# thygate/stable-diffusion-webui-depthmap-script

Measured on NVIDIA H100. Metric: images/sec, higher is better.
Workload: dtype fp16

## Files before the change

### stable-diffusion-webui-depthmap-script_b200/csrc/gemm_wgmma.cu

```cuda
#include <cuda.h>
#include <cuda_fp16.h>
#include <math.h>
#include <stdlib.h>

#include "common.cuh"
#include "tc_common.cuh"

namespace dm {
using namespace tc;

enum GemmEpi : int {
    EPI_STORE_F16 = 0,
    EPI_RESID_F32 = 1,
    EPI_PIXSHUF = 2,
    EPI_HEAD = 3,
    EPI_STORE_F32 = 4,
};
enum GemmAct : int { ACT_NONE = 0, ACT_GELU = 1, ACT_RELU = 2 };

struct GemmParams {
    int M, N, K;
    int epi, act;
    const float *bias;
    __half *C; int ldc;
    __half *C2;
    const __half *R; int ldr;
    const __half *R2; int ldr2;
    float *X; int ldx;
    const float *gamma;
    float head_b2;
    int ps_s, ps_cout, ps_h, ps_w;
    int cB, cH, cW, cCin, hbox, wbox, tiles_x, tiles_y;
    int m_tiles, n_tiles, group_m;
    int corg;
    const float *wscale;
};

template <int BM, int BN>
struct GemmCfg {
    static constexpr int BK = 64;
    static constexpr int WM = BM / 64;
    static constexpr int A_BYTES = BM * BK * 2, B_BYTES = BN * BK * 2;
    static constexpr int STAGE_BYTES = A_BYTES + B_BYTES;
    static constexpr int STAGES = (220 * 1024) / STAGE_BYTES < 8 ? (220 * 1024) / STAGE_BYTES : 8;
    static constexpr int SMEM_BYTES = STAGES * STAGE_BYTES + 256 ;
};
constexpr int GEMM_THREADS = 384;
constexpr int SPLIT_PROMOTE = 1;

__device__ __forceinline__ float gelu_erf(float x) {
    const float u = fminf(fabsf(x), 5.75f);
    float q = -2.992472582263872e-05f;
    q = fmaf(q, u, 0.0007398786256089807f);
    q = fmaf(q, u, -0.007977476343512535f);
    q = fmaf(q, u, 0.05323820561170578f);
    q = fmaf(q, u, 0.45891568064689636f);
    q = fmaf(q, u, 1.1511471271514893f);
    float e;
    const float t = fmaf(-u, q, -1.f);
    asm("ex2.approx.ftz.f32 %0, %1;" : "=f"(e) : "f"(t));
    return fmaf(-u, e, fmaxf(x, 0.f));
}

__device__ __forceinline__ void split_store2(__half *dst, int lo_off, float v0, float v1) {
    const __half2 hi = __floats2half2_rn(v0, v1);
    const float2 hf = __half22float2(hi);
    const __half2 lo = __floats2half2_rn(v0 - hf.x, v1 - hf.y);
    *reinterpret_cast<__half2 *>(dst) = hi;
    *reinterpret_cast<__half2 *>(dst + lo_off) = lo;
    *reinterpret_cast<__half2 *>(dst + 2 * lo_off) = hi;
}

template <int BN, int EPI, bool SPLIT = false>
__device__ __forceinline__ void epilogue_fragment(const GemmParams &p, const float (&acc)[BN / 2], const long long (&m)[2], const bool (&row_ok)[2],
                                                  int n_base, int lane) {
    constexpr int JC = 2;
    const int t = lane & 3;
    float head_acc[2] = {0.f, 0.f};
#pragma unroll
    for (int j0 = 0; j0 < BN / 8; j0 += JC) {
        float2 b2[JC], g2[JC], x[JC][2], ws[JC];
        __half2 rv[JC][2], rv2[JC][2], rl[JC][2], rl2[JC][2];
#pragma unroll
        for (int jj = 0; jj < JC; ++jj) {
            const int n = n_base + 8 * (j0 + jj) + 2 * t;
            b2[jj] = make_float2(0.f, 0.f);
            g2[jj] = make_float2(0.f, 0.f);
            if (n >= p.N) continue;
            if (p.bias) b2[jj] = __ldg(reinterpret_cast<const float2 *>(p.bias + n));
            if (SPLIT) ws[jj] = __ldg(reinterpret_cast<const float2 *>(p.wscale + n));
            if (EPI == EPI_RESID_F32 || EPI == EPI_HEAD) g2[jj] = __ldg(reinterpret_cast<const float2 *>(p.gamma + n));
#pragma unroll
            for (int r = 0; r < 2; ++r) {
                if (!row_ok[r]) continue;
                if (EPI == EPI_RESID_F32) x[jj][r] = *reinterpret_cast<const float2 *>(p.X + m[r] * p.ldx + n);
                if (EPI == EPI_STORE_F16 || EPI == EPI_PIXSHUF) {
                    if (p.R) rv[jj][r] = __ldg(reinterpret_cast<const __half2 *>(p.R + m[r] * p.ldr + n));
                    if (p.R2) rv2[jj][r] = __ldg(reinterpret_cast<const __half2 *>(p.R2 + m[r] * p.ldr2 + n));
                    if (SPLIT && p.R) rl[jj][r] = __ldg(reinterpret_cast<const __half2 *>(p.R + m[r] * p.ldr + p.N + n));
                    if (SPLIT && p.R2) rl2[jj][r] = __ldg(reinterpret_cast<const __half2 *>(p.R2 + m[r] * p.ldr2 + p.N + n));
                }
            }
        }
#pragma unroll
        for (int jj = 0; jj < JC; ++jj) {
            const int j = j0 + jj;
            const int n = n_base + 8 * j + 2 * t;
            if (n >= p.N) continue;
#pragma unroll
            for (int r = 0; r < 2; ++r) {
                if (!row_ok[r]) continue;
                float v0, v1;
                if (SPLIT) { v0 = fmaf(acc[4 * j + 2 * r], ws[jj].x, b2[jj].x); v1 = fmaf(acc[4 * j + 2 * r + 1], ws[jj].y, b2[jj].y); }
                else { v0 = acc[4 * j + 2 * r] + b2[jj].x; v1 = acc[4 * j + 2 * r + 1] + b2[jj].y; }
                if (EPI == EPI_RESID_F32) {
                    float2 xv = x[jj][r];
                    xv.x = fmaf(g2[jj].x, v0, xv.x); xv.y = fmaf(g2[jj].y, v1, xv.y);
                    *reinterpret_cast<float2 *>(p.X + m[r] * p.ldx + n) = xv;
                    continue;
                }
                if (EPI == EPI_STORE_F32) {
                    *reinterpret_cast<float2 *>(p.X + m[r] * p.ldx + n) = make_float2(v0, v1);
                    continue;
                }
                if (p.act == ACT_GELU) { v0 = gelu_erf(v0); v1 = gelu_erf(v1); }
                else if (p.act == ACT_RELU) { v0 = fmaxf(v0, 0.f); v1 = fmaxf(v1, 0.f); }
                if (EPI == EPI_HEAD) {
                    head_acc[r] = fmaf(v1, g2[jj].y, fmaf(v0, g2[jj].x, head_acc[r]));
                    continue;
                }
                if (SPLIT) {
                    if (p.R) { const float2 f = __half22float2(rv[jj][r]), l = __half22float2(rl[jj][r]); v0 += f.x + l.x; v1 += f.y + l.y; }
                    if (p.R2) { const float2 f = __half22float2(rv2[jj][r]), l = __half22float2(rl2[jj][r]); v0 += f.x + l.x; v1 += f.y + l.y; }
                    __half *dst;
                    int lo_off;
                    if (EPI == EPI_PIXSHUF) {
                        const int s = p.ps_s, ij = n / p.ps_cout, co = n % p.ps_cout;
                        const int i = ij / s, jx = ij % s;
                        const long long bb = m[r] / ((long long)p.ps_h * p.ps_w);
                        const int rem = (int)(m[r] % ((long long)p.ps_h * p.ps_w));
                        const int y = rem / p.ps_w, xx = rem % p.ps_w;
                        dst = p.C + (((bb * (p.ps_h * s) + (y * s + i)) * (long long)(p.ps_w * s)) + (xx * s + jx)) * (3 * p.ps_cout) + co;
                        lo_off = p.ps_cout;
                    } else {
                        dst = p.C + m[r] * p.ldc + n;
                        lo_off = p.N;
                    }
                    split_store2(dst, lo_off, v0, v1);
                    if (EPI != EPI_PIXSHUF && p.C2) split_store2(p.C2 + m[r] * p.ldc + n, lo_off, fmaxf(v0, 0.f), fmaxf(v1, 0.f));
                    continue;
                }
                if (p.R) { const float2 f = __half22float2(rv[jj][r]); v0 += f.x; v1 += f.y; }
                if (p.R2) { const float2 f = __half22float2(rv2[jj][r]); v0 += f.x; v1 += f.y; }
                const __half2 h2 = __floats2half2_rn(v0, v1);
                if (EPI == EPI_PIXSHUF) {
                    const int s = p.ps_s, ij = n / p.ps_cout, co = n % p.ps_cout;
                    const int i = ij / s, jx = ij % s;
                    const long long bb = m[r] / ((long long)p.ps_h * p.ps_w);
                    const int rem = (int)(m[r] % ((long long)p.ps_h * p.ps_w));
                    const int y = rem / p.ps_w, xx = rem % p.ps_w;
                    *reinterpret_cast<__half2 *>(p.C + (((bb * (p.ps_h * s) + (y * s + i)) * (long long)(p.ps_w * s)) + (xx * s + jx)) * p.ps_cout + co) = h2;
                } else {
                    *reinterpret_cast<__half2 *>(p.C + m[r] * p.ldc + n) = h2;
                    if (p.C2) *reinterpret_cast<__half2 *>(p.C2 + m[r] * p.ldc + n) = __hmax2(h2, __float2half2_rn(0.f));
                }
            }
        }
    }
    if (EPI == EPI_HEAD) {
#pragma unroll
        for (int r = 0; r < 2; ++r) {
            float s = head_acc[r];
            s += __shfl_xor_sync(0xffffffffu, s, 1);
            s += __shfl_xor_sync(0xffffffffu, s, 2);
            if (t == 0 && row_ok[r]) p.X[m[r]] = fmaxf(s + p.head_b2, 0.f);
        }
    }
}

__device__ __forceinline__ void tile_coords(const GemmParams &p, int t, int &m_blk, int &n_blk) {
    const int per_group = p.group_m * p.n_tiles;
    const int g = t / per_group, r = t - g * per_group;
    m_blk = g * p.group_m + r / p.n_tiles;
    n_blk = r % p.n_tiles;
}

__device__ __forceinline__ void conv_origin(const GemmParams &p, int m_blk, int &cb, int &cy0, int &cx0) {
    const int tiles_per_img = p.tiles_x * p.tiles_y;
    cb = m_blk / tiles_per_img;
    const int t = m_blk % tiles_per_img;
    cy0 = (t / p.tiles_x) * p.hbox;
    cx0 = (t % p.tiles_x) * p.wbox;
}

template <int BM, int BN, bool CONV, bool SPLIT>
__device__ __forceinline__ void gemm_body(const CUtensorMap &tmA, const CUtensorMap &tmB, const GemmParams &p) {
    using Cfg = GemmCfg<BM, BN>;
    extern __shared__ __align__(1024) uint8_t smem_raw[];
    uint8_t *smem = smem_raw;
    uint64_t *full = reinterpret_cast<uint64_t *>(smem + Cfg::STAGES * Cfg::STAGE_BYTES);
    uint64_t *empty = full + Cfg::STAGES;

    const int warp = threadIdx.x >> 5, lane = threadIdx.x & 31;
    const int num_kb = CONV ? 9 * (p.cCin / Cfg::BK) : p.K / Cfg::BK;
    const int my_tiles = (p.m_tiles * p.n_tiles - (int)blockIdx.x + (int)gridDim.x - 1) / (int)gridDim.x;

    if (threadIdx.x == 0) {
        prefetch_tmap(&tmA);
        prefetch_tmap(&tmB);
        for (int s = 0; s < Cfg::STAGES; ++s) { mbar_init(&full[s], 1); mbar_init(&empty[s], 4); }
        fence_barrier_init();
    }
    __syncthreads();

    if (warp < 4) {
        setmaxnreg_dec<40>();
        if (threadIdx.x == 0) {
            int stage = 0, phase = 0;
            for (int i = 0; i < my_tiles; ++i) {
                int m_blk, n_blk, cb = 0, cy0 = 0, cx0 = 0;
                tile_coords(p, blockIdx.x + i * gridDim.x, m_blk, n_blk);
                if (CONV) conv_origin(p, m_blk, cb, cy0, cx0);
                for (int kb = 0; kb < num_kb; ++kb) {
                    mbar_wait(&empty[stage], phase ^ 1);
                    uint8_t *sa = smem + stage * Cfg::STAGE_BYTES, *sb = sa + Cfg::A_BYTES;
                    mbar_arrive_expect_tx(&full[stage], Cfg::STAGE_BYTES);
                    if (CONV) {
                        const int cblks = p.cCin / Cfg::BK;
                        const int tap = kb / cblks, cblk = kb % cblks;
                        const int dy = tap / 3 - 1, dx = tap % 3 - 1;
                        tma_load_4d(sa, &tmA, &full[stage], cblk * Cfg::BK, cx0 + dx + p.corg, cy0 + dy + p.corg, cb);
                    } else {
                        tma_load_2d(sa, &tmA, &full[stage], kb * Cfg::BK, m_blk * BM);
                    }
                    tma_load_2d(sb, &tmB, &full[stage], kb * Cfg::BK, n_blk * BN);
                    if (++stage == Cfg::STAGES) { stage = 0; phase ^= 1; }
                }
            }
        }
        return;
    }

    setmaxnreg_inc<232>();
    const int wg = (warp >> 2) - 1;
    float acc[Cfg::WM][BN / 2];
    float sum[Cfg::WM][BN / 2];
    for (int i = wg; i < my_tiles; i += 2) {
        int m_blk, n_blk, cb = 0, cy0 = 0, cx0 = 0;
        tile_coords(p, blockIdx.x + i * gridDim.x, m_blk, n_blk);
        if (CONV) conv_origin(p, m_blk, cb, cy0, cx0);
        const long long q0 = (long long)i * num_kb;
        int stage = (int)(q0 % Cfg::STAGES), phase = (int)((q0 / Cfg::STAGES) & 1), prev = 0;
        if (i > 0) named_bar_sync(1 + wg, 256);
        if (SPLIT) {
#pragma unroll
            for (int h = 0; h < Cfg::WM; ++h)
#pragma unroll
                for (int e = 0; e < BN / 2; ++e) sum[h][e] = 0.f;
        }
        for (int kb = 0; kb < num_kb; ++kb) {
            mbar_wait(&full[stage], phase);
            const uint32_t sa = smem_u32(smem + stage * Cfg::STAGE_BYTES), sb = sa + Cfg::A_BYTES;
            const uint64_t bdesc = make_desc_kmajor_sw128(sb);
            wgmma_fence();
#pragma unroll
            for (int k = 0; k < Cfg::BK / 16; ++k) {
#pragma unroll
                for (int h = 0; h < Cfg::WM; ++h)
                    wgmma_ss<BN>(acc[h], make_desc_kmajor_sw128(sa + h * (64 * 128)) + (uint64_t)(2 * k), bdesc + (uint64_t)(2 * k),
                                 SPLIT ? ((kb % SPLIT_PROMOTE) | k) != 0 : (kb | k) != 0);
            }
            wgmma_commit();
            if (kb > 0) {
                wgmma_wait<1>();
                if (lane == 0) mbar_arrive(&empty[prev]);
            }
            if (SPLIT && ((kb + 1) % SPLIT_PROMOTE == 0 || kb + 1 == num_kb)) {
                wgmma_wait<0>();
#pragma unroll
                for (int h = 0; h < Cfg::WM; ++h)
#pragma unroll
                    for (int e = 0; e < BN / 2; ++e) sum[h][e] = __fadd_rn(sum[h][e], acc[h][e]);
            }
            prev = stage;
            if (++stage == Cfg::STAGES) { stage = 0; phase ^= 1; }
        }
        if (i + 1 < my_tiles) named_bar_arrive(2 - wg, 256);
        wgmma_wait<0>();
        if (lane == 0) mbar_arrive(&empty[prev]);

#pragma unroll
        for (int h = 0; h < Cfg::WM; ++h) {
            long long m[2];
            bool row_ok[2];
#pragma unroll
            for (int r = 0; r < 2; ++r) {
                const int row = h * 64 + (warp & 3) * 16 + (lane >> 2) + 8 * r;
                if (CONV) {
                    const int y = cy0 + row / p.wbox, x = cx0 + row % p.wbox;
                    row_ok[r] = (y < p.cH) && (x < p.cW);
                    m[r] = ((long long)cb * p.cH + y) * p.cW + x;
                } else {
                    m[r] = (long long)m_blk * BM + row;
                    row_ok[r] = m[r] < p.M;
                }
            }
            const float (&res)[BN / 2] = SPLIT ? sum[h] : acc[h];
            switch (p.epi) {
                case EPI_STORE_F16: epilogue_fragment<BN, EPI_STORE_F16, SPLIT>(p, res, m, row_ok, n_blk * BN, lane); break;
                case EPI_RESID_F32: epilogue_fragment<BN, EPI_RESID_F32, SPLIT>(p, res, m, row_ok, n_blk * BN, lane); break;
                case EPI_PIXSHUF: epilogue_fragment<BN, EPI_PIXSHUF, SPLIT>(p, res, m, row_ok, n_blk * BN, lane); break;
                case EPI_HEAD: epilogue_fragment<BN, EPI_HEAD, SPLIT>(p, res, m, row_ok, n_blk * BN, lane); break;
                case EPI_STORE_F32: epilogue_fragment<BN, EPI_STORE_F32, SPLIT>(p, res, m, row_ok, n_blk * BN, lane); break;
            }
        }
    }
}

template <int BM, int BN, bool CONV>
__global__ void __launch_bounds__(GEMM_THREADS, 1) gemm_wgmma_kernel(const __grid_constant__ CUtensorMap tmA,
                                                                     const __grid_constant__ CUtensorMap tmB, GemmParams p) {
    gemm_body<BM, BN, CONV, false>(tmA, tmB, p);
}

template <int BM, int BN, bool CONV>
__global__ void __launch_bounds__(GEMM_THREADS, 1) gemm_split_kernel(const __grid_constant__ CUtensorMap tmA,
                                                                     const __grid_constant__ CUtensorMap tmB, GemmParams p) {
    gemm_body<BM, BN, CONV, true>(tmA, tmB, p);
}

typedef CUresult (*PFN_encodeTiled)(CUtensorMap *, CUtensorMapDataType, cuuint32_t, void *, const cuuint64_t *, const cuuint64_t *,
                                    const cuuint32_t *, const cuuint32_t *, CUtensorMapInterleave, CUtensorMapSwizzle,
                                    CUtensorMapL2promotion, CUtensorMapFloatOOBfill);

static PFN_encodeTiled get_encode() {
    static PFN_encodeTiled fn = nullptr;
    if (!fn) {
        void *p = nullptr;
        cudaDriverEntryPointQueryResult qres;
        if (cudaGetDriverEntryPoint("cuTensorMapEncodeTiled", &p, cudaEnableDefault, &qres) != cudaSuccess || !p) return nullptr;
        fn = (PFN_encodeTiled)p;
    }
    return fn;
}

int make_tmap_2d(CUtensorMap *tm, const void *ptr, uint64_t rows, uint64_t cols, uint64_t ld, uint32_t box_rows, uint32_t box_cols) {
    PFN_encodeTiled enc = get_encode();
    if (!enc) { set_error("cuTensorMapEncodeTiled unavailable"); return DM_E_CUDA; }
    cuuint64_t dims[2] = {cols, rows};
    cuuint64_t strides[1] = {ld * 2};
    cuuint32_t box[2] = {box_cols, box_rows};
    cuuint32_t es[2] = {1, 1};
    CUresult r = enc(tm, CU_TENSOR_MAP_DATA_TYPE_FLOAT16, 2, const_cast<void *>(ptr), dims, strides, box, es, CU_TENSOR_MAP_INTERLEAVE_NONE,
                     CU_TENSOR_MAP_SWIZZLE_128B, CU_TENSOR_MAP_L2_PROMOTION_L2_256B, CU_TENSOR_MAP_FLOAT_OOB_FILL_NONE);
    if (r != CUDA_SUCCESS) { set_error("cuTensorMapEncodeTiled(2d) failed: %d (rows=%llu cols=%llu ld=%llu)", (int)r, (unsigned long long)rows, (unsigned long long)cols, (unsigned long long)ld); return DM_E_CUDA; }
    return DM_OK;
}

int make_tmap_nhwc(CUtensorMap *tm, const void *ptr, uint64_t B, uint64_t H, uint64_t W, uint64_t C, uint32_t hbox, uint32_t wbox) {
    PFN_encodeTiled enc = get_encode();
    if (!enc) { set_error("cuTensorMapEncodeTiled unavailable"); return DM_E_CUDA; }
    cuuint64_t dims[4] = {C, W, H, B};
    cuuint64_t strides[3] = {C * 2, W * C * 2, H * W * C * 2};
    cuuint32_t box[4] = {64, wbox, hbox, 1};
    cuuint32_t es[4] = {1, 1, 1, 1};
    CUresult r = enc(tm, CU_TENSOR_MAP_DATA_TYPE_FLOAT16, 4, const_cast<void *>(ptr), dims, strides, box, es, CU_TENSOR_MAP_INTERLEAVE_NONE,
                     CU_TENSOR_MAP_SWIZZLE_128B, CU_TENSOR_MAP_L2_PROMOTION_L2_256B, CU_TENSOR_MAP_FLOAT_OOB_FILL_NONE);
    if (r != CUDA_SUCCESS) { set_error("cuTensorMapEncodeTiled(4d) failed: %d", (int)r); return DM_E_CUDA; }
    return DM_OK;
}

template <int BM, int BN, bool CONV, bool SPLIT = false>
static int launch_gemm(const CUtensorMap &tmA, const CUtensorMap &tmB, GemmParams p, int m_tiles, cudaStream_t stream) {
    using Cfg = GemmCfg<BM, BN>;
    static PerDeviceFlag configured;
    static PerDeviceAttr sms(cudaDevAttrMultiProcessorCount);
    void (*kernel)(const CUtensorMap, const CUtensorMap, GemmParams);
    if constexpr (SPLIT) kernel = gemm_split_kernel<BM, BN, CONV>;
    else kernel = gemm_wgmma_kernel<BM, BN, CONV>;
    if (!configured.test_and_set())
        DM_CUDA_CHECK(cudaFuncSetAttribute(kernel, cudaFuncAttributeMaxDynamicSharedMemorySize, Cfg::SMEM_BYTES));
    const long long l2_budget = 24ll << 20, w_bytes = 2ll * p.N * p.K, a_panel = 2ll * BM * p.K;
    const long long g = (l2_budget - w_bytes) / a_panel;
    p.m_tiles = m_tiles;
    p.n_tiles = (p.N + BN - 1) / BN;
    p.group_m = (int)(g < 1 ? 1 : (g > m_tiles ? m_tiles : g));
    const int tiles = m_tiles * p.n_tiles;
    const int grid = tiles < sms.get() ? tiles : sms.get();
    kernel<<<grid, GEMM_THREADS, Cfg::SMEM_BYTES, stream>>>(tmA, tmB, p);
    DM_LAUNCH_CHECK(SPLIT ? "gemm_split_kernel" : "gemm_wgmma_kernel");
    return DM_OK;
}

static int check_epilogue_operands(const GemmParams &p, const char *who) {
    auto misaligned = [](const void *q, size_t a) { return q && (reinterpret_cast<uintptr_t>(q) % a) != 0; };
    const bool f32_rows = p.epi == EPI_RESID_F32 || p.epi == EPI_STORE_F32;
    const bool f16_rows = p.epi == EPI_STORE_F16 || p.epi == EPI_PIXSHUF;
    if ((f32_rows && (!p.X || p.ldx % 2)) || (p.epi == EPI_HEAD && !p.X)) { set_error("%s: fp32 output missing or its pitch is odd (ldx=%d)", who, p.ldx); return DM_E_INVALID; }
    if (f16_rows && (!p.C || (p.epi == EPI_STORE_F16 && p.ldc % 2))) { set_error("%s: fp16 output missing or its pitch is odd (ldc=%d)", who, p.ldc); return DM_E_INVALID; }
    if (f16_rows && ((p.R && p.ldr % 2) || (p.R2 && p.ldr2 % 2))) { set_error("%s: residual pitches must be even (ldr=%d ldr2=%d)", who, p.ldr, p.ldr2); return DM_E_INVALID; }
    if (p.epi == EPI_PIXSHUF && (p.ps_s < 1 || p.ps_cout < 2 || p.ps_cout % 2 || p.N != p.ps_s * p.ps_s * p.ps_cout)) {
        set_error("%s: pixel shuffle needs an even channel count and N = s*s*cout (s=%d cout=%d N=%d)", who, p.ps_s, p.ps_cout, p.N);
        return DM_E_INVALID;
    }
    if ((p.epi == EPI_RESID_F32 || p.epi == EPI_HEAD) && !p.gamma) { set_error("%s: gamma is NULL", who); return DM_E_INVALID; }
    if (misaligned(p.bias, 8) || misaligned(p.gamma, 8) || (f32_rows && misaligned(p.X, 8))) { set_error("%s: fp32 operands must be 8-byte aligned", who); return DM_E_INVALID; }
    if (f16_rows && (misaligned(p.C, 4) || misaligned(p.C2, 4) || misaligned(p.R, 4) || misaligned(p.R2, 4))) { set_error("%s: fp16 operands must be 4-byte aligned", who); return DM_E_INVALID; }
    return DM_OK;
}

static int pick_bn(const GemmParams &p) {
    if (p.epi == EPI_HEAD) return 32;
    return p.N % 256 == 0 ? 256 : (p.N % 128 == 0 ? 128 : (p.N % 64 == 0 ? 64 : 32));
}
static int tile_m(int bn) { return bn == 256 ? 64 : 128; }

static int check_split(const GemmParams &p, const char *who) {
    if (!p.wscale || reinterpret_cast<uintptr_t>(p.wscale) % 8) { set_error("%s: wscale missing or not 8-byte aligned", who); return DM_E_INVALID; }
    const bool f16_out = p.epi == EPI_STORE_F16;
    if ((f16_out && p.ldc < 3 * p.N) || (p.R && p.ldr < 3 * p.N) || (p.R2 && p.ldr2 < 3 * p.N)) {
        set_error("%s: split rows need pitches of at least 3N (N=%d ldc=%d ldr=%d ldr2=%d)", who, p.N, p.ldc, p.ldr, p.ldr2);
        return DM_E_INVALID;
    }
    return DM_OK;
}
static int split_bn(const GemmParams &p) { const int bn = pick_bn(p); return bn > 64 ? 64 : bn; }

int gemm_f16(const __half *A, int lda, const __half *W, int ldw, GemmParams p, cudaStream_t stream) {
    if (p.K % 64 != 0 || p.N % 32 != 0) { set_error("gemm_f16: K must be a multiple of 64 and N of 32 (K=%d N=%d)", p.K, p.N); return DM_E_INVALID; }
    if (p.epi == EPI_HEAD && p.N != 32) { set_error("gemm_f16: the fused head needs N = 32 (N=%d)", p.N); return DM_E_UNSUPPORTED; }
    if (int rc0 = check_epilogue_operands(p, "gemm_f16")) return rc0;
    if ((lda % 8) || (ldw % 8)) { set_error("gemm_f16: row pitches must be multiples of 8 elements"); return DM_E_INVALID; }
    const int bn = pick_bn(p), bm = tile_m(bn);
    const int m_tiles = (p.M + bm - 1) / bm;
    CUtensorMap tmA, tmB;
    int rc = make_tmap_2d(&tmA, A, (uint64_t)p.M, (uint64_t)p.K, (uint64_t)lda, (uint32_t)bm, 64);
    if (rc) return rc;
    rc = make_tmap_2d(&tmB, W, (uint64_t)p.N, (uint64_t)p.K, (uint64_t)ldw, (uint32_t)bn, 64);
    if (rc) return rc;
    switch (bn) {
        case 256: return launch_gemm<64, 256, false>(tmA, tmB, p, m_tiles, stream);
        case 128: return launch_gemm<128, 128, false>(tmA, tmB, p, m_tiles, stream);
        case 64: return launch_gemm<128, 64, false>(tmA, tmB, p, m_tiles, stream);
        case 32: return launch_gemm<128, 32, false>(tmA, tmB, p, m_tiles, stream);
    }
    set_error("gemm_f16: unsupported N tile %d", bn);
    return DM_E_UNSUPPORTED;
}

int gemm_split(const __half *A, int lda, const __half *W, int ldw, GemmParams p, cudaStream_t stream) {
    if (p.K % 64 != 0 || p.N % 32 != 0) { set_error("gemm_split: K must be a multiple of 64 and N of 32 (K=%d N=%d)", p.K, p.N); return DM_E_INVALID; }
    if (p.epi == EPI_HEAD && p.N != 32) { set_error("gemm_split: the fused head needs N = 32 (N=%d)", p.N); return DM_E_UNSUPPORTED; }
    if (int rc0 = check_epilogue_operands(p, "gemm_split")) return rc0;
    if (int rc0 = check_split(p, "gemm_split")) return rc0;
    if ((lda % 8) || (ldw % 8)) { set_error("gemm_split: row pitches must be multiples of 8 elements"); return DM_E_INVALID; }
    const int bn = split_bn(p);
    const int m_tiles = (p.M + 127) / 128;
    CUtensorMap tmA, tmB;
    int rc = make_tmap_2d(&tmA, A, (uint64_t)p.M, (uint64_t)p.K, (uint64_t)lda, 128, 64);
    if (rc) return rc;
    rc = make_tmap_2d(&tmB, W, (uint64_t)p.N, (uint64_t)p.K, (uint64_t)ldw, (uint32_t)bn, 64);
    if (rc) return rc;
    return bn == 64 ? launch_gemm<128, 64, false, true>(tmA, tmB, p, m_tiles, stream) : launch_gemm<128, 32, false, true>(tmA, tmB, p, m_tiles, stream);
}

static int conv3x3_launch(const __half *src, int halo, int B, int H, int W, int Cin, const __half *Wt, GemmParams p, cudaStream_t stream,
                          bool split = false) {
    const int bn = split ? split_bn(p) : pick_bn(p), bm = tile_m(bn);
    int best_w = bm; double best_eff = -1;
    for (int wb = bm; wb >= 8; wb >>= 1) {
        const int hb = bm / wb;
        const double eff = (double)(W * H) / ((double)((W + wb - 1) / wb * wb) * ((H + hb - 1) / hb * hb));
        if (eff > best_eff + 1e-9) { best_eff = eff; best_w = wb; }
    }
    p.wbox = best_w; p.hbox = bm / best_w;
    p.tiles_x = (W + p.wbox - 1) / p.wbox; p.tiles_y = (H + p.hbox - 1) / p.hbox;
    p.cB = B; p.cH = H; p.cW = W; p.cCin = Cin; p.corg = halo;
    p.M = B * H * W; p.K = 9 * Cin;
    const int m_tiles = B * p.tiles_x * p.tiles_y;
    CUtensorMap tmA, tmB;
    int rc = make_tmap_nhwc(&tmA, src, B, H + 2 * halo, W + 2 * halo, Cin, p.hbox, p.wbox);
    if (rc) return rc;
    rc = make_tmap_2d(&tmB, Wt, (uint64_t)p.N, (uint64_t)p.K, (uint64_t)p.K, (uint32_t)bn, 64);
    if (rc) return rc;
    if (split) return bn == 64 ? launch_gemm<128, 64, true, true>(tmA, tmB, p, m_tiles, stream) : launch_gemm<128, 32, true, true>(tmA, tmB, p, m_tiles, stream);
    switch (bn) {
        case 256: return launch_gemm<64, 256, true>(tmA, tmB, p, m_tiles, stream);
        case 128: return launch_gemm<128, 128, true>(tmA, tmB, p, m_tiles, stream);
        case 64: return launch_gemm<128, 64, true>(tmA, tmB, p, m_tiles, stream);
        case 32: return launch_gemm<128, 32, true>(tmA, tmB, p, m_tiles, stream);
    }
    set_error("conv3x3_f16: unsupported N tile %d", bn);
    return DM_E_UNSUPPORTED;
}

static int check_conv3x3(const GemmParams &p, int Cin, const char *who) {
    if (Cin % 64 != 0 || p.N % 32 != 0) { set_error("%s: Cin must be a multiple of 64 and Cout of 32", who); return DM_E_INVALID; }
    if (p.epi == EPI_HEAD && p.N != 32) { set_error("%s: the fused head needs Cout = 32 (Cout=%d)", who, p.N); return DM_E_UNSUPPORTED; }
    return check_epilogue_operands(p, who);
}

int conv3x3_f16(const __half *act, int B, int H, int W, int Cin, const __half *Wt, GemmParams p, cudaStream_t stream) {
    if (int rc = check_conv3x3(p, Cin, "conv3x3_f16")) return rc;
    return conv3x3_launch(act, 0, B, H, W, Cin, Wt, p, stream);
}

__global__ void __launch_bounds__(256) conv_halo_circular_kernel(const __half *__restrict__ act, int B, int H, int W, int C, __half *__restrict__ halo) {
    const int c8 = C / 8;
    const long long total = (long long)B * (H + 2) * (W + 2) * c8;
    for (long long i = (long long)blockIdx.x * blockDim.x + threadIdx.x; i < total; i += (long long)gridDim.x * blockDim.x) {
        const int c = (int)(i % c8) * 8;
        long long r = i / c8;
        const int x = (int)(r % (W + 2));
        r /= W + 2;
        const int y = (int)(r % (H + 2));
        const long long b = r / (H + 2);
        const int sy = wrap_index(y - 1, H), sx = wrap_index(x - 1, W);
        reinterpret_cast<uint4 *>(halo)[i] = __ldg(reinterpret_cast<const uint4 *>(act + ((b * H + sy) * W + sx) * C + c));
    }
}

int conv_halo_circular(const __half *act, int B, int H, int W, int C, __half *halo, cudaStream_t stream) {
    if (!act || !halo || B <= 0 || H <= 0 || W <= 0 || C <= 0 || C % 8) { set_error("dm_circular_halo_f16: bad arguments (C must be a positive multiple of 8)"); return DM_E_INVALID; }
    if ((reinterpret_cast<uintptr_t>(act) | reinterpret_cast<uintptr_t>(halo)) % 16) { set_error("dm_circular_halo_f16: tensors must be 16-byte aligned"); return DM_E_INVALID; }
    static PerDeviceAttr sms(cudaDevAttrMultiProcessorCount);
    const long long total = (long long)B * (H + 2) * (W + 2) * (C / 8);
    const long long blocks = (total + 255) / 256, cap = 16ll * sms.get();
    conv_halo_circular_kernel<<<(unsigned)(blocks < cap ? blocks : cap), 256, 0, stream>>>(act, B, H, W, C, halo);
    DM_LAUNCH_CHECK("conv_halo_circular_kernel");
    return DM_OK;
}

int conv3x3_circular_f16(const __half *act, __half *halo, int B, int H, int W, int Cin, const __half *Wt, GemmParams p, cudaStream_t stream) {
    if (int rc = check_conv3x3(p, Cin, "conv3x3_circular")) return rc;
    if (int rc = conv_halo_circular(act, B, H, W, Cin, halo, stream)) return rc;
    return conv3x3_launch(halo, 1, B, H, W, Cin, Wt, p, stream);
}

int conv3x3_split(const __half *act, __half *halo, int B, int H, int W, int Cin, const __half *Wt, GemmParams p, cudaStream_t stream) {
    if (int rc = check_conv3x3(p, Cin, "conv3x3_split")) return rc;
    if (int rc = check_split(p, "conv3x3_split")) return rc;
    if (!halo) return conv3x3_launch(act, 0, B, H, W, 3 * Cin, Wt, p, stream, true);
    if (int rc = conv_halo_circular(act, B, H, W, 3 * Cin, halo, stream)) return rc;
    return conv3x3_launch(halo, 1, B, H, W, 3 * Cin, Wt, p, stream, true);
}

}

extern "C" __attribute__((visibility("default"))) int dm_gemm_f16(const void *A, int lda, const void *W, int ldw, const float *bias, void *C,
                                                               int ldc, int M, int N, int K, int act, int out_f32, void *stream) {
    using namespace dm;
    GemmParams p;
    memset(&p, 0, sizeof(p));
    p.M = M; p.N = N; p.K = K; p.act = act; p.bias = bias;
    if (out_f32) { p.epi = EPI_STORE_F32; p.X = (float *)C; p.ldx = ldc; }
    else { p.epi = EPI_STORE_F16; p.C = (__half *)C; p.ldc = ldc; }
    return gemm_f16((const __half *)A, lda, (const __half *)W, ldw, p, (cudaStream_t)stream);
}

extern "C" __attribute__((visibility("default"))) int dm_conv3x3_f16(const void *act, int B, int H, int W, int Cin, const void *Wt, const float *bias,
                                                                  void *out, int Cout, int relu, void *stream) {
    using namespace dm;
    GemmParams p;
    memset(&p, 0, sizeof(p));
    p.N = Cout; p.act = relu ? ACT_RELU : ACT_NONE; p.bias = bias; p.epi = EPI_STORE_F16; p.C = (__half *)out; p.ldc = Cout;
    return conv3x3_f16((const __half *)act, B, H, W, Cin, (const __half *)Wt, p, (cudaStream_t)stream);
}

static void desc_to_params(const dm_gemm_desc *d, dm::GemmParams &p) {
    memset(&p, 0, sizeof(p));
    p.M = d->M; p.N = d->N; p.K = d->K; p.epi = d->epi; p.act = d->act; p.bias = d->bias;
    p.C = (__half *)d->C; p.ldc = d->ldc; p.C2 = (__half *)d->C2;
    p.R = (const __half *)d->R; p.ldr = d->ldr; p.R2 = (const __half *)d->R2; p.ldr2 = d->ldr2;
    p.X = d->X; p.ldx = d->ldx; p.gamma = d->gamma; p.head_b2 = d->head_b2;
    p.ps_s = d->ps_s; p.ps_cout = d->ps_cout; p.ps_h = d->ps_h; p.ps_w = d->ps_w;
}

extern "C" __attribute__((visibility("default"))) int dm_gemm_ex(const void *A, int lda, const void *W, int ldw, const dm_gemm_desc *d, void *stream) {
    if (!A || !W || !d) { dm::set_error("dm_gemm_ex: null argument"); return DM_E_INVALID; }
    dm::GemmParams p;
    desc_to_params(d, p);
    return dm::gemm_f16((const __half *)A, lda, (const __half *)W, ldw, p, (cudaStream_t)stream);
}

extern "C" __attribute__((visibility("default"))) int dm_conv3x3_ex(const void *act, int B, int H, int W, int Cin, const void *Wt, const dm_gemm_desc *d, void *stream) {
    if (!act || !Wt || !d) { dm::set_error("dm_conv3x3_ex: null argument"); return DM_E_INVALID; }
    dm::GemmParams p;
    desc_to_params(d, p);
    return dm::conv3x3_f16((const __half *)act, B, H, W, Cin, (const __half *)Wt, p, (cudaStream_t)stream);
}

extern "C" __attribute__((visibility("default"))) int dm_circular_halo_f16(const void *act, int B, int H, int W, int C, void *halo, void *stream) {
    return dm::conv_halo_circular((const __half *)act, B, H, W, C, (__half *)halo, (cudaStream_t)stream);
}

extern "C" __attribute__((visibility("default"))) int dm_conv3x3_circular_ex(const void *act, void *halo, int B, int H, int W, int Cin, const void *Wt,
                                                                          const dm_gemm_desc *d, void *stream) {
    if (!act || !halo || !Wt || !d) { dm::set_error("dm_conv3x3_circular_ex: null argument"); return DM_E_INVALID; }
    dm::GemmParams p;
    desc_to_params(d, p);
    return dm::conv3x3_circular_f16((const __half *)act, (__half *)halo, B, H, W, Cin, (const __half *)Wt, p, (cudaStream_t)stream);
}

extern "C" __attribute__((visibility("default"))) int dm_gemm_split_ex(const void *A, int lda, const void *W, int ldw, const float *wscale,
                                                                    const dm_gemm_desc *d, void *stream) {
    if (!A || !W || !d) { dm::set_error("dm_gemm_split_ex: null argument"); return DM_E_INVALID; }
    dm::GemmParams p;
    desc_to_params(d, p);
    p.wscale = wscale;
    return dm::gemm_split((const __half *)A, lda, (const __half *)W, ldw, p, (cudaStream_t)stream);
}

extern "C" __attribute__((visibility("default"))) int dm_conv3x3_split_ex(const void *act, void *halo, int B, int H, int W, int Cin, const void *Wt,
                                                                       const float *wscale, const dm_gemm_desc *d, void *stream) {
    if (!act || !Wt || !d) { dm::set_error("dm_conv3x3_split_ex: null argument"); return DM_E_INVALID; }
    dm::GemmParams p;
    desc_to_params(d, p);
    p.wscale = wscale;
    return dm::conv3x3_split((const __half *)act, (__half *)halo, B, H, W, Cin, (const __half *)Wt, p, (cudaStream_t)stream);
}
```

Baseline: 319.5.

## Stage GEMM epilogue through shared memory for coalesced row-contiguous stores

```diff
diff --git a/stable-diffusion-webui-depthmap-script_b200/csrc/gemm_wgmma.cu b/stable-diffusion-webui-depthmap-script_b200/csrc/gemm_wgmma.cu
--- a/stable-diffusion-webui-depthmap-script_b200/csrc/gemm_wgmma.cu
+++ b/stable-diffusion-webui-depthmap-script_b200/csrc/gemm_wgmma.cu
@@ -36,14 +36,19 @@
     const float *wscale;
 };
 
+constexpr int EPI_COLS = 32;
+constexpr int EPI_PITCH = EPI_COLS + 8;
+
 template <int BM, int BN>
 struct GemmCfg {
     static constexpr int BK = 64;
     static constexpr int WM = BM / 64;
     static constexpr int A_BYTES = BM * BK * 2, B_BYTES = BN * BK * 2;
     static constexpr int STAGE_BYTES = A_BYTES + B_BYTES;
-    static constexpr int STAGES = (220 * 1024) / STAGE_BYTES < 8 ? (220 * 1024) / STAGE_BYTES : 8;
-    static constexpr int SMEM_BYTES = STAGES * STAGE_BYTES + 256 ;
+    static constexpr int STAGING_BYTES = 2 * 64 * EPI_PITCH * 4;
+    static constexpr int RING_BUDGET = 220 * 1024 - STAGING_BYTES;
+    static constexpr int STAGES = RING_BUDGET / STAGE_BYTES < 8 ? RING_BUDGET / STAGE_BYTES : 8;
+    static constexpr int SMEM_BYTES = STAGES * STAGE_BYTES + 256  + STAGING_BYTES;
 };
 constexpr int GEMM_THREADS = 384;
 constexpr int SPLIT_PROMOTE = 1;
@@ -71,110 +76,135 @@
     *reinterpret_cast<__half2 *>(dst + 2 * lo_off) = hi;
 }
 
-template <int BN, int EPI, bool SPLIT = false>
-__device__ __forceinline__ void epilogue_fragment(const GemmParams &p, const float (&acc)[BN / 2], const long long (&m)[2], const bool (&row_ok)[2],
-                                                  int n_base, int lane) {
-    constexpr int JC = 2;
-    const int t = lane & 3;
-    float head_acc[2] = {0.f, 0.f};
-#pragma unroll
-    for (int j0 = 0; j0 < BN / 8; j0 += JC) {
-        float2 b2[JC], g2[JC], x[JC][2], ws[JC];
-        __half2 rv[JC][2], rv2[JC][2], rl[JC][2], rl2[JC][2];
-#pragma unroll
-        for (int jj = 0; jj < JC; ++jj) {
-            const int n = n_base + 8 * (j0 + jj) + 2 * t;
-            b2[jj] = make_float2(0.f, 0.f);
-            g2[jj] = make_float2(0.f, 0.f);
-            if (n >= p.N) continue;
-            if (p.bias) b2[jj] = __ldg(reinterpret_cast<const float2 *>(p.bias + n));
-            if (SPLIT) ws[jj] = __ldg(reinterpret_cast<const float2 *>(p.wscale + n));
-            if (EPI == EPI_RESID_F32 || EPI == EPI_HEAD) g2[jj] = __ldg(reinterpret_cast<const float2 *>(p.gamma + n));
-#pragma unroll
-            for (int r = 0; r < 2; ++r) {
-                if (!row_ok[r]) continue;
-                if (EPI == EPI_RESID_F32) x[jj][r] = *reinterpret_cast<const float2 *>(p.X + m[r] * p.ldx + n);
+template <int BN, int EPI, bool SPLIT>
+__device__ __forceinline__ void epilogue_staged(const GemmParams &p, const float (&acc)[BN / 2], float *stage, const int (&m)[8], unsigned ok,
+                                                int n_base, int wg) {
+    const int tid = threadIdx.x & 127, lane = tid & 31;
+    const int wrow = (tid >> 5) * 16 + (lane >> 2), wcol = 2 * (lane & 3);
+    const int rrow = tid >> 4, c2 = 2 * (tid & 15);
+    constexpr int NS = BN / EPI_COLS;
+#pragma unroll 1
+    for (int s = 0; s < NS; ++s) {
+        if (n_base + s * EPI_COLS >= p.N) break;
+#pragma unroll
+        for (int ss = 0; ss < NS; ++ss) {
+            if (ss != s) continue;
+#pragma unroll
+            for (int jj = 0; jj < EPI_COLS / 8; ++jj) {
+                const int j = ss * (EPI_COLS / 8) + jj;
+#pragma unroll
+                for (int r = 0; r < 2; ++r)
+                    *reinterpret_cast<float2 *>(stage + (wrow + 8 * r) * EPI_PITCH + 8 * jj + wcol) = make_float2(acc[4 * j + 2 * r], acc[4 * j + 2 * r + 1]);
+            }
+        }
+        named_bar_sync(3 + wg, 128);
+
+        const int n = n_base + s * EPI_COLS + c2;
+        float2 b2 = make_float2(0.f, 0.f), g2 = make_float2(0.f, 0.f), ws = make_float2(1.f, 1.f);
+        if (p.bias) b2 = __ldg(reinterpret_cast<const float2 *>(p.bias + n));
+        if (SPLIT) ws = __ldg(reinterpret_cast<const float2 *>(p.wscale + n));
+        if (EPI == EPI_RESID_F32) g2 = __ldg(reinterpret_cast<const float2 *>(p.gamma + n));
+        int pcol = 0, co = 0;
+        if (EPI == EPI_PIXSHUF) {
+            const int ij = n / p.ps_cout;
+            co = n % p.ps_cout;
+            pcol = (ij / p.ps_s) * (p.ps_w * p.ps_s) + ij % p.ps_s;
+        }
+#pragma unroll
+        for (int k0 = 0; k0 < 8; k0 += 4) {
+            float2 x[8];
+            __half2 rv[8], rv2[8], rl[8], rl2[8];
+#pragma unroll
+            for (int k = k0; k < k0 + 4; ++k) {
+                if (!((ok >> k) & 1)) continue;
+                if (EPI == EPI_RESID_F32) x[k] = *reinterpret_cast<const float2 *>(p.X + (long long)m[k] * p.ldx + n);
                 if (EPI == EPI_STORE_F16 || EPI == EPI_PIXSHUF) {
-                    if (p.R) rv[jj][r] = __ldg(reinterpret_cast<const __half2 *>(p.R + m[r] * p.ldr + n));
-                    if (p.R2) rv2[jj][r] = __ldg(reinterpret_cast<const __half2 *>(p.R2 + m[r] * p.ldr2 + n));
-                    if (SPLIT && p.R) rl[jj][r] = __ldg(reinterpret_cast<const __half2 *>(p.R + m[r] * p.ldr + p.N + n));
-                    if (SPLIT && p.R2) rl2[jj][r] = __ldg(reinterpret_cast<const __half2 *>(p.R2 + m[r] * p.ldr2 + p.N + n));
+                    if (p.R) rv[k] = __ldg(reinterpret_cast<const __half2 *>(p.R + (long long)m[k] * p.ldr + n));
+                    if (p.R2) rv2[k] = __ldg(reinterpret_cast<const __half2 *>(p.R2 + (long long)m[k] * p.ldr2 + n));
+                    if (SPLIT && p.R) rl[k] = __ldg(reinterpret_cast<const __half2 *>(p.R + (long long)m[k] * p.ldr + p.N + n));
+                    if (SPLIT && p.R2) rl2[k] = __ldg(reinterpret_cast<const __half2 *>(p.R2 + (long long)m[k] * p.ldr2 + p.N + n));
                 }
             }
-        }
-#pragma unroll
-        for (int jj = 0; jj < JC; ++jj) {
-            const int j = j0 + jj;
-            const int n = n_base + 8 * j + 2 * t;
-            if (n >= p.N) continue;
-#pragma unroll
-            for (int r = 0; r < 2; ++r) {
-                if (!row_ok[r]) continue;
+#pragma unroll
+            for (int k = k0; k < k0 + 4; ++k) {
+                if (!((ok >> k) & 1)) continue;
+                const float2 a = *reinterpret_cast<const float2 *>(stage + (rrow + 8 * k) * EPI_PITCH + c2);
+                long long pix = 0;
+                if (EPI == EPI_PIXSHUF) {
+                    const int hw = p.ps_h * p.ps_w, bb = m[k] / hw, rem = m[k] - bb * hw, y = rem / p.ps_w, xx = rem - y * p.ps_w;
+                    pix = ((long long)bb * (p.ps_h * p.ps_s) + y * p.ps_s) * (long long)(p.ps_w * p.ps_s) + xx * p.ps_s + pcol;
+                }
                 float v0, v1;
-                if (SPLIT) { v0 = fmaf(acc[4 * j + 2 * r], ws[jj].x, b2[jj].x); v1 = fmaf(acc[4 * j + 2 * r + 1], ws[jj].y, b2[jj].y); }
-                else { v0 = acc[4 * j + 2 * r] + b2[jj].x; v1 = acc[4 * j + 2 * r + 1] + b2[jj].y; }
+                if (SPLIT) { v0 = fmaf(a.x, ws.x, b2.x); v1 = fmaf(a.y, ws.y, b2.y); }
+                else { v0 = a.x + b2.x; v1 = a.y + b2.y; }
                 if (EPI == EPI_RESID_F32) {
-                    float2 xv = x[jj][r];
-                    xv.x = fmaf(g2[jj].x, v0, xv.x); xv.y = fmaf(g2[jj].y, v1, xv.y);
-                    *reinterpret_cast<float2 *>(p.X + m[r] * p.ldx + n) = xv;
+                    float2 xv = x[k];
+                    xv.x = fmaf(g2.x, v0, xv.x); xv.y = fmaf(g2.y, v1, xv.y);
+                    *reinterpret_cast<float2 *>(p.X + (long long)m[k] * p.ldx + n) = xv;
                     continue;
                 }
                 if (EPI == EPI_STORE_F32) {
-                    *reinterpret_cast<float2 *>(p.X + m[r] * p.ldx + n) = make_float2(v0, v1);
+                    *reinterpret_cast<float2 *>(p.X + (long long)m[k] * p.ldx + n) = make_float2(v0, v1);
                     continue;
                 }
                 if (p.act == ACT_GELU) { v0 = gelu_erf(v0); v1 = gelu_erf(v1); }
                 else if (p.act == ACT_RELU) { v0 = fmaxf(v0, 0.f); v1 = fmaxf(v1, 0.f); }
-                if (EPI == EPI_HEAD) {
-                    head_acc[r] = fmaf(v1, g2[jj].y, fmaf(v0, g2[jj].x, head_acc[r]));
+                if (SPLIT) {
+                    if (p.R) { const float2 f = __half22float2(rv[k]), l = __half22float2(rl[k]); v0 += f.x + l.x; v1 += f.y + l.y; }
+                    if (p.R2) { const float2 f = __half22float2(rv2[k]), l = __half22float2(rl2[k]); v0 += f.x + l.x; v1 += f.y + l.y; }
+                    if (EPI == EPI_PIXSHUF) {
+                        split_store2(p.C + pix * (3 * p.ps_cout) + co, p.ps_cout, v0, v1);
+                    } else {
+                        split_store2(p.C + (long long)m[k] * p.ldc + n, p.N, v0, v1);
+                        if (p.C2) split_store2(p.C2 + (long long)m[k] * p.ldc + n, p.N, fmaxf(v0, 0.f), fmaxf(v1, 0.f));
+                    }
                     continue;
                 }
-                if (SPLIT) {
-                    if (p.R) { const float2 f = __half22float2(rv[jj][r]), l = __half22float2(rl[jj][r]); v0 += f.x + l.x; v1 += f.y + l.y; }
-                    if (p.R2) { const float2 f = __half22float2(rv2[jj][r]), l = __half22float2(rl2[jj][r]); v0 += f.x + l.x; v1 += f.y + l.y; }
-                    __half *dst;
-                    int lo_off;
-                    if (EPI == EPI_PIXSHUF) {
-                        const int s = p.ps_s, ij = n / p.ps_cout, co = n % p.ps_cout;
-                        const int i = ij / s, jx = ij % s;
-                        const long long bb = m[r] / ((long long)p.ps_h * p.ps_w);
-                        const int rem = (int)(m[r] % ((long long)p.ps_h * p.ps_w));
-                        const int y = rem / p.ps_w, xx = rem % p.ps_w;
-                        dst = p.C + (((bb * (p.ps_h * s) + (y * s + i)) * (long long)(p.ps_w * s)) + (xx * s + jx)) * (3 * p.ps_cout) + co;
-                        lo_off = p.ps_cout;
-                    } else {
-                        dst = p.C + m[r] * p.ldc + n;
-                        lo_off = p.N;
-                    }
-                    split_store2(dst, lo_off, v0, v1);
-                    if (EPI != EPI_PIXSHUF && p.C2) split_store2(p.C2 + m[r] * p.ldc + n, lo_off, fmaxf(v0, 0.f), fmaxf(v1, 0.f));
-                    continue;
-                }
-                if (p.R) { const float2 f = __half22float2(rv[jj][r]); v0 += f.x; v1 += f.y; }
-                if (p.R2) { const float2 f = __half22float2(rv2[jj][r]); v0 += f.x; v1 += f.y; }
+                if (p.R) { const float2 f = __half22float2(rv[k]); v0 += f.x; v1 += f.y; }
+                if (p.R2) { const float2 f = __half22float2(rv2[k]); v0 += f.x; v1 += f.y; }
                 const __half2 h2 = __floats2half2_rn(v0, v1);
                 if (EPI == EPI_PIXSHUF) {
-                    const int s = p.ps_s, ij = n / p.ps_cout, co = n % p.ps_cout;
-                    const int i = ij / s, jx = ij % s;
-                    const long long bb = m[r] / ((long long)p.ps_h * p.ps_w);
-                    const int rem = (int)(m[r] % ((long long)p.ps_h * p.ps_w));
-                    const int y = rem / p.ps_w, xx = rem % p.ps_w;
-                    *reinterpret_cast<__half2 *>(p.C + (((bb * (p.ps_h * s) + (y * s + i)) * (long long)(p.ps_w * s)) + (xx * s + jx)) * p.ps_cout + co) = h2;
+                    *reinterpret_cast<__half2 *>(p.C + pix * p.ps_cout + co) = h2;
                 } else {
-                    *reinterpret_cast<__half2 *>(p.C + m[r] * p.ldc + n) = h2;
-                    if (p.C2) *reinterpret_cast<__half2 *>(p.C2 + m[r] * p.ldc + n) = __hmax2(h2, __float2half2_rn(0.f));
+                    *reinterpret_cast<__half2 *>(p.C + (long long)m[k] * p.ldc + n) = h2;
+                    if (p.C2) *reinterpret_cast<__half2 *>(p.C2 + (long long)m[k] * p.ldc + n) = __hmax2(h2, __float2half2_rn(0.f));
                 }
             }
         }
-    }
-    if (EPI == EPI_HEAD) {
+        named_bar_sync(3 + wg, 128);
+    }
+}
+
+template <int BN, bool SPLIT>
+__device__ __forceinline__ void epilogue_head(const GemmParams &p, const float (&acc)[BN / 2], const long long (&m)[2], const bool (&row_ok)[2],
+                                              int n_base, int lane) {
+    const int t = lane & 3;
+    float head_acc[2] = {0.f, 0.f};
+#pragma unroll
+    for (int j = 0; j < BN / 8; ++j) {
+        const int n = n_base + 8 * j + 2 * t;
+        if (n >= p.N) continue;
+        float2 b2 = make_float2(0.f, 0.f), ws;
+        if (p.bias) b2 = __ldg(reinterpret_cast<const float2 *>(p.bias + n));
+        if (SPLIT) ws = __ldg(reinterpret_cast<const float2 *>(p.wscale + n));
+        const float2 g2 = __ldg(reinterpret_cast<const float2 *>(p.gamma + n));
 #pragma unroll
         for (int r = 0; r < 2; ++r) {
-            float s = head_acc[r];
-            s += __shfl_xor_sync(0xffffffffu, s, 1);
-            s += __shfl_xor_sync(0xffffffffu, s, 2);
-            if (t == 0 && row_ok[r]) p.X[m[r]] = fmaxf(s + p.head_b2, 0.f);
-        }
+            if (!row_ok[r]) continue;
+            float v0, v1;
+            if (SPLIT) { v0 = fmaf(acc[4 * j + 2 * r], ws.x, b2.x); v1 = fmaf(acc[4 * j + 2 * r + 1], ws.y, b2.y); }
+            else { v0 = acc[4 * j + 2 * r] + b2.x; v1 = acc[4 * j + 2 * r + 1] + b2.y; }
+            if (p.act == ACT_GELU) { v0 = gelu_erf(v0); v1 = gelu_erf(v1); }
+            else if (p.act == ACT_RELU) { v0 = fmaxf(v0, 0.f); v1 = fmaxf(v1, 0.f); }
+            head_acc[r] = fmaf(v1, g2.y, fmaf(v0, g2.x, head_acc[r]));
+        }
+    }
+#pragma unroll
+    for (int r = 0; r < 2; ++r) {
+        float s = head_acc[r];
+        s += __shfl_xor_sync(0xffffffffu, s, 1);
+        s += __shfl_xor_sync(0xffffffffu, s, 2);
+        if (t == 0 && row_ok[r]) p.X[m[r]] = fmaxf(s + p.head_b2, 0.f);
     }
 }
 
@@ -243,6 +273,7 @@
 
     setmaxnreg_inc<232>();
     const int wg = (warp >> 2) - 1;
+    float *staging = reinterpret_cast<float *>(smem + Cfg::STAGES * Cfg::STAGE_BYTES + 256) + wg * 64 * EPI_PITCH;
     float acc[Cfg::WM][BN / 2];
     float sum[Cfg::WM][BN / 2];
     for (int i = wg; i < my_tiles; i += 2) {
@@ -289,29 +320,39 @@
         wgmma_wait<0>();
         if (lane == 0) mbar_arrive(&empty[prev]);
 
+        auto tile_row = [&](int row, long long &m) -> bool {
+            if (CONV) {
+                const int y = cy0 + row / p.wbox, x = cx0 + row % p.wbox;
+                m = ((long long)cb * p.cH + y) * p.cW + x;
+                return y < p.cH && x < p.cW;
+            }
+            m = (long long)m_blk * BM + row;
+            return m < p.M;
+        };
 #pragma unroll
         for (int h = 0; h < Cfg::WM; ++h) {
-            long long m[2];
-            bool row_ok[2];
-#pragma unroll
-            for (int r = 0; r < 2; ++r) {
-                const int row = h * 64 + (warp & 3) * 16 + (lane >> 2) + 8 * r;
-                if (CONV) {
-                    const int y = cy0 + row / p.wbox, x = cx0 + row % p.wbox;
-                    row_ok[r] = (y < p.cH) && (x < p.cW);
-                    m[r] = ((long long)cb * p.cH + y) * p.cW + x;
-                } else {
-                    m[r] = (long long)m_blk * BM + row;
-                    row_ok[r] = m[r] < p.M;
-                }
-            }
             const float (&res)[BN / 2] = SPLIT ? sum[h] : acc[h];
+            if (p.epi == EPI_HEAD) {
+                long long m[2];
+                bool row_ok[2];
+#pragma unroll
+                for (int r = 0; r < 2; ++r) row_ok[r] = tile_row(h * 64 + (warp & 3) * 16 + (lane >> 2) + 8 * r, m[r]);
+                epilogue_head<BN, SPLIT>(p, res, m, row_ok, n_blk * BN, lane);
+                continue;
+            }
+            int m[8];
+            unsigned ok = 0;
+#pragma unroll
+            for (int k = 0; k < 8; ++k) {
+                long long mk;
+                ok |= (unsigned)tile_row(h * 64 + ((threadIdx.x & 127) >> 4) + 8 * k, mk) << k;
+                m[k] = (int)mk;
+            }
             switch (p.epi) {
-                case EPI_STORE_F16: epilogue_fragment<BN, EPI_STORE_F16, SPLIT>(p, res, m, row_ok, n_blk * BN, lane); break;
-                case EPI_RESID_F32: epilogue_fragment<BN, EPI_RESID_F32, SPLIT>(p, res, m, row_ok, n_blk * BN, lane); break;
-                case EPI_PIXSHUF: epilogue_fragment<BN, EPI_PIXSHUF, SPLIT>(p, res, m, row_ok, n_blk * BN, lane); break;
-                case EPI_HEAD: epilogue_fragment<BN, EPI_HEAD, SPLIT>(p, res, m, row_ok, n_blk * BN, lane); break;
-                case EPI_STORE_F32: epilogue_fragment<BN, EPI_STORE_F32, SPLIT>(p, res, m, row_ok, n_blk * BN, lane); break;
+                case EPI_STORE_F16: epilogue_staged<BN, EPI_STORE_F16, SPLIT>(p, res, staging, m, ok, n_blk * BN, wg); break;
+                case EPI_RESID_F32: epilogue_staged<BN, EPI_RESID_F32, SPLIT>(p, res, staging, m, ok, n_blk * BN, wg); break;
+                case EPI_PIXSHUF: epilogue_staged<BN, EPI_PIXSHUF, SPLIT>(p, res, staging, m, ok, n_blk * BN, wg); break;
+                case EPI_STORE_F32: epilogue_staged<BN, EPI_STORE_F32, SPLIT>(p, res, staging, m, ok, n_blk * BN, wg); break;
             }
         }
     }
```

New measurement: 345.7, median of 6. 8.2% higher.
